# brunothg/sfm-mvs-pipeline

Measured on AMD Instinct MI355X. Metric: descriptor-pairs/s matched, higher is better.
Workload: dtype int8->int32 (exact; f32 in/out); 1 GPU; 50 images x 8192 SIFT-128 f32, unordered all-pairs (1225 pairs); descriptors_per_image=8192, pairs=1225, parallelism=pair-sharded x1

## Files before the change

sfm-mvs-pipeline_amd/csrc/match_device.hpp:

```cpp
#pragma once
#include <hip/hip_runtime.h>
#include <cstdint>
#include <climits>
#include <cstdlib>
#include "match_common.hpp"
#include "sift_fp6.hpp"

namespace sfmx {

typedef int i32x4 __attribute__((ext_vector_type(4)));
typedef int i32x16 __attribute__((ext_vector_type(16)));
typedef unsigned u32x4 __attribute__((ext_vector_type(4)));
typedef int i32x8 __attribute__((ext_vector_type(8)));
typedef float f32x4 __attribute__((ext_vector_type(4)));
typedef float f32x16 __attribute__((ext_vector_type(16)));

#define GLOBAL_AS __attribute__((address_space(1)))
#define LDS_AS __attribute__((address_space(3)))

__device__ __forceinline__ int med3i(int a, int b, int c) { return max(min(a, b), min(max(a, b), c)); }
__device__ __forceinline__ int v_med3(int a, int b, int c) {
    int d;
    asm("v_med3_i32 %0, %1, %2, %3" : "=v"(d) : "v"(a), "v"(b), "v"(c));
    return d;
// ... 154 lines not shown
            }
        }
        if ((s % SPC) == SPC - 1 || s + 1 == nstages) {
            const int cb = (s / SPC) * 256;
#pragma unroll
            for (int qt = 0; qt < QT; ++qt) {
                const int p1 = __shfl_xor(c1[qt], 32), p2 = __shfl_xor(c2[qt], 32);
                const int m1 = max(c1[qt], p1), m2 = max(min(c1[qt], p1), max(c2[qt], p2));
#pragma unroll
                for (int e = 0; e < 2; ++e) {
                    const int key = e == 0 ? m1 : m2;
                    if (key != INT_MIN) {
                        const int t_ = -(key >> 8), j_ = cb + 255 - (key & 255);
                        if (t_ < T2[qt]) {
                            if (t_ < T1[qt]) { T2[qt] = T1[qt]; J2[qt] = J1[qt]; T1[qt] = t_; J1[qt] = j_; }
                            else { T2[qt] = t_; J2[qt] = j_; }
                        }
                    }
                }
                c1[qt] = c2[qt] = INT_MIN;
            }
        }
        asm volatile("s_waitcnt vmcnt(0)" ::: "memory");
        __syncthreads();
    }

#pragma unroll
    for (int qt = 0; qt < QT; ++qt) {
        const int qi = qrow[qt];
        if (h != 0 || qi < 0) continue;
        if constexpr (LISTS) {
            const long long na = norm[L.row0 + qi];
            const unsigned long long k1 = T1[qt] != INT_MAX ? ((unsigned long long)(na + T1[qt]) << 32) | (unsigned)J1[qt] : ~0ull;
            const unsigned long long k2 = T2[qt] != INT_MAX ? ((unsigned long long)(na + T2[qt]) << 32) | (unsigned)J2[qt] : ~0ull;
            *reinterpret_cast<ulonglong2*>(top2 + 2 * (P.dense_base + qslot[qt])) = make_ulonglong2(k1, k2);
            continue;
        }
        const int64_t o = P.dense_base + qi;
        if (nt == 0) { out_idx[o] = -1; out_dist[o] = 0.f; continue; }
        const int64_t na = norm[L.row0 + qi];
        const int64_t s1 = (int64_t)T1[qt] + na, s2 = (int64_t)T2[qt] + na;
        if (nt >= 2 && s2 >= SQRT_SAFE) {
            const int slot = atomicAdd(slow_count, 1);
            slow_list[slot] = make_int2(w.pair, qi);
            out_idx[o] = -2;
            continue;
        }
        const float d1 = sqrt_rn_int(s1);
        out_idx[o] = lowe_select(J1[qt], d1, nt >= 2 ? sqrt_rn_int(s2) : 0.f, nt, ratio);
        out_dist[o] = d1;
    }
}

template <int QT, int WAVES, int MINW, int STAGE, bool MFMA_FIRST, bool GATHER = false, bool LISTS = false, bool VIA = false>
__global__ __launch_bounds__(WAVES * 64, MINW)
void sift_knn2_kernel(const WorkItem* __restrict__ work, const PairDev* __restrict__ pairs,
                      const ImgDev* __restrict__ imgs, const int8_t* __restrict__ desc8,
                      const int32_t* __restrict__ norm, const int32_t* __restrict__ keyc,
                      int32_t* __restrict__ out_idx, float* __restrict__ out_dist,
                      int2* __restrict__ slow_list, int32_t* __restrict__ slow_count, double ratio,
                      const int32_t* __restrict__ qlist = nullptr, const int32_t* __restrict__ qcount = nullptr,
                      const int32_t* __restrict__ work2_n = nullptr, unsigned long long* __restrict__ top2 = nullptr,
                      const int32_t* __restrict__ via = nullptr) {
#define SIFT_KNN2_ITEM(item, nwork)                                                                                    \
    sift_knn2_item<QT, WAVES, MINW, STAGE, MFMA_FIRST, GATHER, LISTS, VIA>(                                            \
        item, nwork, work, pairs, imgs, desc8, norm, keyc, out_idx, out_dist, slow_list, slow_count, ratio, qlist, qcount, \
        top2, via)
    if constexpr (VIA) {
        const int nwork = *work2_n;
        for (int item = blockIdx.x; item < nwork; item += gridDim.x) SIFT_KNN2_ITEM(item, nwork);
    } else if constexpr (GATHER) {
        const int nwork = *work2_n;
        if ((int)blockIdx.x < nwork) SIFT_KNN2_ITEM((int)blockIdx.x, nwork);
    } else {
        SIFT_KNN2_ITEM((int)blockIdx.x, (int)gridDim.x);
    }
#undef SIFT_KNN2_ITEM
}

__device__ __forceinline__ int xcd_ticket(int32_t* ticket, int n) {
    const int x0 = (int)(__builtin_amdgcn_s_getreg(0x1814) & 7);
    for (int k = 0; k < 8; ++k) {
        const int x = (x0 + k) & 7, b0 = (int)((int64_t)n * x / 8), b1 = (int)((int64_t)n * (x + 1) / 8);
        if (b1 <= b0) continue;
        if (__hip_atomic_load(&ticket[x], __ATOMIC_RELAXED, __HIP_MEMORY_SCOPE_AGENT) >= b1 - b0) continue;
        const int t = atomicAdd(&ticket[x], 1);
        if (t < b1 - b0) return b0 + t;
    }
    return -1;
}

template <bool CERT>
__device__ __forceinline__ void screen6_forward(float k1, float k2, int r1, int qi, int nt, int2 q2, int emax2, int amax2,
                                                double ratio, int pair, int64_t dense_base, int32_t* __restrict__ qlist,
                                                int32_t* __restrict__ qcount, int32_t* __restrict__ qmask,
                                                unsigned long long* __restrict__ top2, int32_t* __restrict__ qlist2,
                                                int32_t* __restrict__ qcount2) {
    const int usable = (int)(nt >= 2) & (int)(k2 > fp6::KEY_VALID);
    const int rej = usable & fp6::certainly_rejected(k1, k2, q2.x, q2.y, emax2, amax2, ratio);
    if (rej == 0) {
        const int64_t slot = dense_base + atomicAdd(&qcount[pair], 1);
        qlist[slot] = qi;
        if constexpr (CERT) {
            const int cert = fp6::certified(k1, k2, r1, nt, q2.x, q2.y, emax2, amax2, ratio);
            qmask[slot] = cert ? 1 << r1 : QMASK_FULL_ROUTE;
            if (!cert) qlist2[dense_base + atomicAdd(&qcount2[pair], 1)] = (int32_t)(slot - dense_base);
        } else {
            qmask[slot] = 0xFFFF;
        }
        top2[2 * slot] = ~0ull;
        top2[2 * slot + 1] = ~0ull;
    }
}

template <int STAGE>
struct Screen6Stage {
    static constexpr int WAVES = 4;
    static constexpr int A_BYTES = STAGE * 64, B_BYTES = STAGE * 32;
    static constexpr int GA = A_BYTES / (WAVES * 64 * 16), GB = B_BYTES / (WAVES * 64 * 16), GK = STAGE / 64;
    static constexpr int BUF_BYTES = A_BYTES + B_BYTES + STAGE * 4;
    static_assert(STAGE % 128 == 0 && ROW_ALIGN % STAGE == 0, "whole DMA instructions per wave; stages inside the padded rows");
    __amdgpu_buffer_rsrc_t rows, keys;
    int va, vb, vk;
    int wid;

    __device__ __forceinline__ Screen6Stage(const uint32_t* __restrict__ desc6, const float* __restrict__ keyf, const ImgDev& R) {
        const int tid = threadIdx.x;
        wid = __builtin_amdgcn_readfirstlane(tid >> 6);
        const int ra = tid >> 2, rb = tid >> 1;
        va = ra * fp6::ROW_BYTES + 16 * ((tid & 3) ^ fp6::swz_a(ra));
        vb = rb * fp6::ROW_BYTES + 64 + 16 * ((tid & 1) ^ fp6::swz_b(rb));
        vk = (tid & 63) * 4;
        rows = __builtin_amdgcn_make_buffer_rsrc(const_cast<uint32_t*>(desc6 + R.row0 * fp6::ROW_WORDS), 0,
                                                 R.rows_pad * fp6::ROW_BYTES, 0x00020000);
        keys = __builtin_amdgcn_make_buffer_rsrc(const_cast<float*>(keyf + R.row0), 0, R.rows_pad * 4, 0x00020000);
    }
    __device__ __forceinline__ void issue(char* lds, int s, int buf) const {
        char* base = lds + buf * BUF_BYTES;
        const int row0 = s * STAGE;
#pragma unroll
        for (int i = 0; i < GA; ++i)
            __builtin_amdgcn_raw_ptr_buffer_load_lds(rows, (LDS_AS void*)(base + (i * WAVES + wid) * 1024), 16, va,
                                                     (row0 + i * 64) * fp6::ROW_BYTES, 0, 0);
#pragma unroll
        for (int i = 0; i < GB; ++i)
            __builtin_amdgcn_raw_ptr_buffer_load_lds(rows, (LDS_AS void*)(base + A_BYTES + (i * WAVES + wid) * 1024), 16, vb,
                                                     (row0 + i * 128) * fp6::ROW_BYTES, 0, 0);
        if (wid < GK)
            __builtin_amdgcn_raw_ptr_buffer_load_lds(keys, (LDS_AS void*)(base + A_BYTES + B_BYTES + wid * 256), 4, vk,
                                                     (row0 + wid * 64) * 4, 0, 0);
    }
};

template <int QT, int WAVES, int MINW, int STAGE, bool CERT>
__global__ __launch_bounds__(WAVES * 64, MINW)
void sift_screen6_kernel(const WorkItem* __restrict__ work, const PairDev* __restrict__ pairs,
                         const ImgDev* __restrict__ imgs, const uint32_t* __restrict__ desc6,
                         const float* __restrict__ keyf, const int2* __restrict__ ne,
                         const int32_t* __restrict__ imax,
                         int32_t* __restrict__ qlist, int32_t* __restrict__ qcount, double ratio,
                         int32_t* __restrict__ qmask, unsigned long long* __restrict__ top2,
                         int32_t* __restrict__ qlist2, int32_t* __restrict__ qcount2) {
    static_assert(QT * WAVES * 16 == 512, "work items are 512 queries");
    using Stage = Screen6Stage<STAGE>;
    static_assert(WAVES == Stage::WAVES, "whole DMA instructions per wave");
    constexpr int A_BYTES = Stage::A_BYTES, B_BYTES = Stage::B_BYTES, BUF_BYTES = Stage::BUF_BYTES;
    __shared__ __attribute__((aligned(16))) char lds[2 * BUF_BYTES];

    const int lane = threadIdx.x & 63, g = lane >> 4, l16 = lane & 15;
    const WorkItem w = work[xcd_remap(blockIdx.x, gridDim.x)];
    const PairDev P = pairs[w.pair];
    const ImgDev L = imgs[P.left], R = imgs[P.right];
    const int nq = L.rows, nt = R.rows;
    const Stage stager(desc6, keyf, R);
    const int wid = stager.wid;
    const int qbase = w.q0 + wid * (QT * 16);

    i32x8 bq[QT];
#pragma unroll
    for (int qt = 0; qt < QT; ++qt) {
        const uint32_t* src = desc6 + (L.row0 + qbase + qt * 16 + l16) * fp6::ROW_WORDS;
        const i32x4 lo = *reinterpret_cast<const i32x4*>(src + 4 * g);
        const int2 hi = *reinterpret_cast<const int2*>(src + 16 + 2 * g);
        bq[qt] = i32x8{lo.x, lo.y, lo.z, lo.w, hi.x, hi.y, 0, 0};
    }
    float ch[QT][4];
#pragma unroll
    for (int qt = 0; qt < QT; ++qt)
#pragma unroll
        for (int i = 0; i < 4; ++i) ch[qt][i] = fp6::KEY_INIT;

    const int nstages = (nt + STAGE - 1) / STAGE;
    const char* ra = lds + l16 * 64 + 16 * (g ^ fp6::swz_a(l16));
    const char* rb = lds + A_BYTES + l16 * 32 + 16 * ((g >> 1) ^ fp6::swz_b(l16)) + 8 * (g & 1);
    const char* rk = lds + A_BYTES + B_BYTES + 16 * g;
    static_assert(fp6::swz_a(16) == fp6::swz_a(0) && fp6::swz_b(16) == fp6::swz_b(0), "swizzle period of 16 rows");

    if (nstages > 0) stager.issue(lds, 0, 0);
    asm volatile("s_waitcnt vmcnt(0)" ::: "memory");
    __syncthreads();
    for (int s = 0; s < nstages; ++s) {
        const int buf = s & 1;
        if (s + 1 < nstages) stager.issue(lds, s + 1, buf ^ 1);
        const char *pa = ra + buf * BUF_BYTES, *pb = rb + buf * BUF_BYTES, *pk = rk + buf * BUF_BYTES;
#pragma unroll
        for (int t = 0; t < STAGE / 32; ++t) {
            i32x8 a[2];
            f32x4 cinit[2];
#pragma unroll
            for (int b = 0; b < 2; ++b) {
                const int blk = 2 * t + b;
                const i32x4 lo = *reinterpret_cast<const i32x4*>(pa + blk * 16 * 64);
                const long long hi = *(const volatile LDS_AS long long*)(pb + blk * 16 * 32);
                a[b] = i32x8{lo.x, lo.y, lo.z, lo.w, (int)hi, (int)(hi >> 32), 0, 0};
                cinit[b] = *reinterpret_cast<const f32x4*>(pk + blk * 16 * 4);
            }
#pragma unroll
            for (int qt = 0; qt < QT; ++qt) {
                const f32x4 acc0 = fp6::mfma16<fp6::FMT_E2M3, false>(a[0], bq[qt], cinit[0]);
                const f32x4 acc1 = fp6::mfma16<fp6::FMT_E2M3, false>(a[1], bq[qt], cinit[1]);
#pragma unroll
                for (int i = 0; i < 4; ++i) ch[qt][i] = fmaxf(fmaxf(ch[qt][i], acc0[i]), acc1[i]);
            }
        }
        asm volatile("s_waitcnt vmcnt(0)" ::: "memory");
        __syncthreads();
    }

    const int emax2 = imax[2 * P.right], amax2 = imax[2 * P.right + 1];
    static_assert(QT % 4 == 0, "four tiles per decision pass");
    float kk1[4] = {}, kk2[4] = {};
    int rr1[4] = {};
#pragma unroll
    for (int qt = 0; qt < QT; ++qt) {
        float k1 = fp6::KEY_INIT, k2 = fp6::KEY_INIT;
        int r1 = 4 * g;
#pragma unroll
        for (int i = 0; i < 4; ++i) {
            const float v = ch[qt][i];
            if constexpr (CERT) r1 = v > k1 ? 4 * g + i : r1;
            k2 = fmaxf(k2, fminf(k1, v));
            k1 = fmaxf(k1, v);
        }
#pragma unroll
        for (int o = 16; o <= 32; o <<= 1) {
            const float p1 = __shfl_xor(k1, o), p2 = __shfl_xor(k2, o);
            if constexpr (CERT) {
                const int pr = __shfl_xor(r1, o);
                r1 = p1 > k1 ? pr : r1;
            }
            k2 = fmaxf(fminf(k1, p1), fmaxf(k2, p2));
            k1 = fmaxf(k1, p1);
        }
        kk1[qt & 3] = k1; kk2[qt & 3] = k2; rr1[qt & 3] = r1;
        if ((qt & 3) != 3) continue;
        k1 = kk1[0]; k2 = kk2[0]; r1 = rr1[0];
#pragma unroll
        for (int j = 1; j < 4; ++j) {
            k1 = g == j ? kk1[j] : k1;
            k2 = g == j ? kk2[j] : k2;
            r1 = g == j ? rr1[j] : r1;
        }
        const int qi = qbase + ((qt & ~3) + g) * 16 + l16;
        if (qi >= nq || nt == 0) continue;
        screen6_forward<CERT>(k1, k2, r1, qi, nt, ne[L.row0 + qi], emax2, amax2, ratio, w.pair, P.dense_base, qlist, qcount,
                              qmask, top2, qlist2, qcount2);
    }
}

constexpr int SIFT_RIDE_MAX = 32;

template <int QTMAX>
__global__ __launch_bounds__(256, 4)
void sift_rows_kernel(const PairDev* __restrict__ pairs, const ImgDev* __restrict__ imgs,
                      const int8_t* __restrict__ desc8, const int32_t* __restrict__ norm,
                      const int32_t* __restrict__ qlist, const int32_t* __restrict__ qmask,
                      const int32_t* __restrict__ qcount, const int32_t* __restrict__ qcount2,
                      const int32_t* __restrict__ porder, unsigned long long* __restrict__ top2) {
    constexpr int WIN = 1024;
    constexpr int EPT = WIN / 256;
    constexpr int RIDER = 1 << 30;
    constexpr int TILE = 32 * SIFT_DIM;
    __shared__ __attribute__((aligned(16))) char rows_lds[4][2][TILE];
    __shared__ int nrm_lds[4][2][64];
    __shared__ int pool[WIN];
    __shared__ __attribute__((aligned(16))) int strip[4][32];
    __shared__ int s_cnt[5];
    static_assert(sizeof(rows_lds) + sizeof(nrm_lds) + sizeof(pool) + sizeof(strip) + sizeof(s_cnt) <= 160 * 1024 / 4,
                  "pass-2 LDS must leave four workgroups resident per CU");

    const int tid = threadIdx.x, lane = tid & 63, h = lane >> 5, l32 = lane & 31;
    const int wid = __builtin_amdgcn_readfirstlane(tid >> 6);
    const int item = xcd_remap(blockIdx.x, gridDim.x);
    const int pi = porder[item >> 2], G = item & 3, r = 4 * G + wid;
    const int cnt = qcount[pi];
    if (cnt == 0) return;
    const PairDev P = pairs[pi];
    const ImgDev L = imgs[P.left], R = imgs[P.right];
    const int nt = R.rows;
    if (4 * G >= nt) return;
    const bool live = r < nt;
    const int ntile = R.rows_pad >> 9;
    const int32_t* qls = qlist + P.dense_base;
    const int32_t* qms = qmask + P.dense_base;
    const bool riders = qcount2[pi] <= SIFT_RIDE_MAX;

    const int8_t* rbase = desc8 + (R.row0 + r) * SIFT_DIM;
    const int32_t* nbase = norm + R.row0 + r;
    auto stage = [&](int t, int b) {
        const int8_t* src = rbase + (int64_t)t * (32 * 16 * SIFT_DIM);
#pragma unroll
        for (int u = 0; u < 4; ++u) {
            const int rr = 8 * u + (lane >> 3), c = (lane & 7) ^ ((rr >> 1) & 7);
            __builtin_amdgcn_global_load_lds((const GLOBAL_AS void*)(src + (unsigned)(rr * (16 * SIFT_DIM) + 16 * c)),
                                             (LDS_AS void*)(&rows_lds[wid][b][u * 1024]), 16, 0, 0);
        }
        __builtin_amdgcn_global_load_lds((const GLOBAL_AS void*)(nbase + t * (32 * 16) + 16 * l32),
                                         (LDS_AS void*)(&nrm_lds[wid][b][0]), 4, 0, 0);
    };
    int cur = 0;
    if (live) stage(0, 0);

    for (int e0 = 0; e0 < cnt; e0 += WIN) {
        if (tid < 5) s_cnt[tid] = 0;
        __syncthreads();
        int ent[EPT], at[EPT], li[EPT];
#pragma unroll
        for (int k = 0; k < EPT; ++k) {
            const int e = e0 + k * 256 + tid;
            li[k] = -1;
            ent[k] = at[k] = 0;
            if (e < cnt) {
                const int mk = qms[e];
                if (mk & QMASK_FULL_ROUTE) li[k] = riders ? 4 : -1;
                else if (mk != 0 && ((__ffs(mk) - 1) >> 2) == G) li[k] = (__ffs(mk) - 1) & 3;
                if (li[k] >= 0) {
                    ent[k] = qls[e] | ((e - e0) << 20) | (li[k] == 4 ? RIDER : 0);
                    at[k] = atomicAdd(&s_cnt[li[k]], 1);
                }
            }
        }
        __syncthreads();
        int base[5], n_l[5];
        base[0] = 0;
#pragma unroll
        for (int l = 0; l < 5; ++l) {
            n_l[l] = __builtin_amdgcn_readfirstlane(s_cnt[l]);
            if (l < 4) base[l + 1] = base[l] + n_l[l];
        }
#pragma unroll
        for (int k = 0; k < EPT; ++k)
            if (li[k] >= 0) pool[base[li[k]] + at[k]] = ent[k];
        __syncthreads();
        const int n_own = n_l[wid], b_own = base[wid], n = live ? n_own + n_l[4] : 0;
        for (int g0 = 0; g0 < n; g0 += 32 * QTMAX) {
            const int nqt = min(QTMAX, (n - g0 + 31) >> 5);
            auto entry = [&](int qt) {
                const int qe = g0 + qt * 32 + l32;
                return qe < n ? (qe < n_own ? pool[b_own + qe] : pool[base[4] + qe - n_own]) : -1;
            };
            i32x4 bq[QTMAX][4];
#pragma unroll
            for (int qt = 0; qt < QTMAX; ++qt) {
#pragma unroll
                for (int m = 0; m < 4; ++m) bq[qt][m] = i32x4{0, 0, 0, 0};
                if (qt < nqt) {
                    const int qpk = entry(qt);
                    const int64_t lrow = L.row0 + (qpk < 0 ? 0 : (qpk & 0xFFFFF));
                    const i32x4* src = reinterpret_cast<const i32x4*>(desc8 + lrow * SIFT_DIM);
#pragma unroll
                    for (int m = 0; m < 4; ++m) bq[qt][m] = src[2 * m + h];
                }
            }
            int T1[QTMAX], T2[QTMAX], c1[QTMAX], c2[QTMAX];
            unsigned JJ[QTMAX];
#pragma unroll
            for (int qt = 0; qt < QTMAX; ++qt) {
                T1[qt] = T2[qt] = INT_MAX; JJ[qt] = 0; c1[qt] = c2[qt] = INT_MIN;
            }
            for (int t = 0; t < ntile; ++t) {
// ... 317 lines not shown
```

sfm-mvs-pipeline_amd/csrc/match_diag.hip:

```cpp
#ifdef SFMX_DIAG
#include "match_device.hpp"
#include "diag.hpp"

namespace sfmx {

__global__ void prep_hamming_kernel(const uint8_t* __restrict__ src, int rows, int cols, int rows_pad,
                                    uint8_t* __restrict__ dst) {
    const int64_t i = (int64_t)blockIdx.x * blockDim.x + threadIdx.x;
    const int64_t total = (int64_t)rows_pad * ORB_BYTES;
    if (i >= total) return;
    const int r = (int)(i / ORB_BYTES), c = (int)(i % ORB_BYTES);
    dst[i] = (r < rows && c < cols) ? src[(int64_t)r * cols + c] : 0;
}

template <int QT, int WAVES, int MINW, int STAGE>
__global__ __launch_bounds__(WAVES * 64, MINW)
void sift_screen_kernel(const WorkItem* __restrict__ work, const PairDev* __restrict__ pairs,
                        const ImgDev* __restrict__ imgs, const int8_t* __restrict__ desc8,
                        const int32_t* __restrict__ norm, const int32_t* __restrict__ keyc2,
                        int32_t* __restrict__ out_idx, float* __restrict__ out_dist,
                        int32_t* __restrict__ qlist, int32_t* __restrict__ qcount, double ratio) {
    constexpr int GLDS = STAGE * SIFT_DIM / (WAVES * 64 * 16);
    static_assert(GLDS * WAVES * 64 * 16 == STAGE * SIFT_DIM, "stage must split into whole 16-B pieces");
    constexpr int DESC_BYTES = STAGE * SIFT_DIM;
// ... 872 lines not shown
                    for (int r = 0; r < 4; r += 2) {
                        const float ka = acc[b][r], kb = acc[b][r + 1];
                        c2[qt] = fmaxf(__builtin_amdgcn_fmed3f(c1[qt], ka, kb), c2[qt]);
                        c1[qt] = fmaxf(c1[qt], fmaxf(ka, kb));
                    }
            }
        }
        if ((s % SPC) == SPC - 1 || s + 1 == nstages) {
            const int cb = (s / SPC) * CHUNK;
#pragma unroll
            for (int qt = 0; qt < QT; ++qt) {
                float m1 = c1[qt], m2 = c2[qt];
#pragma unroll
                for (int o = 16; o <= 32; o <<= 1) {
                    const float p1 = __shfl_xor(m1, o), p2 = __shfl_xor(m2, o);
                    m2 = fmaxf(fminf(m1, p1), fmaxf(m2, p2));
                    m1 = fmaxf(m1, p1);
                }
#pragma unroll
                for (int e = 0; e < 2; ++e) {
                    const float v = e == 0 ? m1 : m2;
                    if (v >= KEY_FLOOR) {
                        const float ip = __builtin_floorf(v);
                        const int dot = (int)ip - 767;
                        const int t_ = (256 - dot) >> 1;
                        const int j_ = cb + 16383 - (int)((v - ip) * 16384.0f);
                        if (t_ < T2[qt]) {
                            if (t_ < T1[qt]) { T2[qt] = T1[qt]; J2[qt] = J1[qt]; T1[qt] = t_; J1[qt] = j_; }
                            else { T2[qt] = t_; J2[qt] = j_; }
                        }
                    }
                }
                c1[qt] = c2[qt] = 0.f;
            }
        }
        asm volatile("s_waitcnt vmcnt(0)" ::: "memory");
        __syncthreads();
    }
#pragma unroll
    for (int qt = 0; qt < QT; ++qt) {
        const int qi = qrow[qt];
        if (g != 0 || qi < 0) continue;
        const int64_t o = P.dense_base + qi;
        if (nt == 0) { out_idx[o] = -1; out_dist[o] = 0.f; continue; }
        const float d1 = (float)T1[qt], d2 = (float)T2[qt];
        out_idx[o] = lowe_select(J1[qt], d1, d2, nt, ratio);
        out_dist[o] = d1;
    }
}

template <int QPL>
__global__ __launch_bounds__(256, 2)
void orb_knn2_kernel(const WorkItem* __restrict__ work, const PairDev* __restrict__ pairs,
                     const ImgDev* __restrict__ imgs, const uint8_t* __restrict__ desc8,
                     int32_t* __restrict__ out_idx, float* __restrict__ out_dist, double ratio) {
    constexpr int STAGE = 256;
    constexpr int BUF = STAGE * ORB_BYTES;
    __shared__ __attribute__((aligned(16))) uint8_t lds[2 * BUF];
    const int wid = threadIdx.x >> 6;
    const WorkItem w = work[xcd_remap(blockIdx.x, gridDim.x)];
    const PairDev P = pairs[w.pair];
    const ImgDev L = imgs[P.left], R = imgs[P.right];
    const int nq = L.rows, nt = R.rows;

    u32x4 q[QPL][2];
#pragma unroll
    for (int e = 0; e < QPL; ++e) {
        const int qi = w.q0 + e * 256 + threadIdx.x;
        const u32x4* src = reinterpret_cast<const u32x4*>(desc8 + (L.row0 + qi) * ORB_BYTES);
        q[e][0] = src[0]; q[e][1] = src[1];
    }
    unsigned b1[QPL], b2[QPL];
#pragma unroll
    for (int e = 0; e < QPL; ++e) b1[e] = b2[e] = 0xffffffffu;

    const uint8_t* tbase = desc8 + R.row0 * ORB_BYTES;
    const int nstages = (nt + STAGE - 1) / STAGE;
    auto stage = [&](int s, int buf) {
        uint8_t* base = lds + buf * BUF;
#pragma unroll
        for (int i = 0; i < 2; ++i) {
            const uint8_t* g = tbase + (int64_t)s * BUF + i * 4096 + threadIdx.x * 16;
            __builtin_amdgcn_global_load_lds((const GLOBAL_AS void*)g, (LDS_AS void*)(base + i * 4096 + wid * 1024), 16, 0, 0);
        }
    };
    if (nstages > 0) stage(0, 0);
    asm volatile("s_waitcnt vmcnt(0)" ::: "memory");
    __syncthreads();
    for (int s = 0; s < nstages; ++s) {
        const int buf = s & 1;
        if (s + 1 < nstages) stage(s + 1, buf ^ 1);
        const u32x4* tl = reinterpret_cast<const u32x4*>(lds + buf * BUF);
        const int lim = min(STAGE, nt - s * STAGE);
        const unsigned j0 = (unsigned)(s * STAGE);
        for (int jj = 0; jj < lim; ++jj) {
            const u32x4 t0 = tl[2 * jj], t1 = tl[2 * jj + 1];
#pragma unroll
            for (int e = 0; e < QPL; ++e) {
                unsigned d = __builtin_popcount(q[e][0].x ^ t0.x);
                d += __builtin_popcount(q[e][0].y ^ t0.y);
                d += __builtin_popcount(q[e][0].z ^ t0.z);
                d += __builtin_popcount(q[e][0].w ^ t0.w);
                d += __builtin_popcount(q[e][1].x ^ t1.x);
                d += __builtin_popcount(q[e][1].y ^ t1.y);
                d += __builtin_popcount(q[e][1].z ^ t1.z);
                d += __builtin_popcount(q[e][1].w ^ t1.w);
                const unsigned key = (d << 23) | (j0 + jj);
                b2[e] = med3u(b1[e], b2[e], key);
                b1[e] = min(b1[e], key);
            }
        }
        asm volatile("s_waitcnt vmcnt(0)" ::: "memory");
        __syncthreads();
    }
#pragma unroll
    for (int e = 0; e < QPL; ++e) {
        const int qi = w.q0 + e * 256 + threadIdx.x;
        if (qi >= nq) continue;
        const int64_t o = P.dense_base + qi;
        if (nt == 0) { out_idx[o] = -1; out_dist[o] = 0.f; continue; }
        const float d1 = (float)(b1[e] >> 23), d2 = (float)(b2[e] >> 23);
        out_idx[o] = lowe_select((int)(b1[e] & 0x7fffffu), d1, d2, nt, ratio);
        out_dist[o] = d1;
    }
}

hipError_t launch_prep_hamming(const uint8_t* src, int rows, int cols, int rows_pad, uint8_t* dst, hipStream_t st) {
    const int64_t total = (int64_t)rows_pad * ORB_BYTES;
    if (total == 0) return hipSuccess;
    prep_hamming_kernel<<<(unsigned)((total + 255) / 256), 256, 0, st>>>(src, rows, cols, rows_pad, dst);
    return hipGetLastError();
}
#define RECORD_SCREEN()                                              \
    if (ev_screen) {    \
        const hipError_t e_ = hipEventRecord(ev_screen, st);         \
        if (e_ != hipSuccess) return e_;                             \
    }

hipError_t launch_sift_diag(const MatchRoute& r, const MatchBufs& b, int n_work, int n_pairs, double ratio, hipStream_t st,
                            hipEvent_t ev_screen) {
    if (r.sift_product()) return launch_sift_product(b, n_work, n_pairs, ratio, r.full_row_grid, st, ev_screen);
    if (n_work == 0) return hipSuccess;
    using R = MatchRoute;
    int32_t* qlist2 = reinterpret_cast<int32_t*>(b.slot1);
    int32_t* qcount2 = b.qcount + arena_qcount2(n_pairs);
    if (r.sift_lists) {
        switch (r.pass2) {
        case R::ROWS:
        case R::SUBSET_CERT:
            if (r.screen == R::FP6_32)
                sift_screen6w_kernel<4, 2, 128, true><<<n_work, 256, 0, st>>>(b.work, b.pairs, b.imgs, b.desc6, b.keyf, b.ne, b.imax,
                                                                             b.qlist, b.qcount, ratio, b.qmask, b.top2, qlist2, qcount2);
            else
                sift_screen6_kernel<8, 4, 2, 128, true><<<n_work, 256, 0, st>>>(b.work, b.pairs, b.imgs, b.desc6, b.keyf, b.ne, b.imax,
                                                                               b.qlist, b.qcount, ratio, b.qmask, b.top2, qlist2, qcount2);
            RECORD_SCREEN();
            if (r.pass2 == R::SUBSET_CERT)
                sift_subset_kernel<4, true><<<n_pairs * 16, 256, 0, st>>>(b.pairs, b.imgs, b.desc8, b.norm, b.qlist, b.qmask, b.qcount,
                                                                          b.porder, b.top2, b.slot1, qcount2, SIFT_RIDE_MAX);
            else
                sift_rows_kernel<2><<<n_pairs * 4, 256, 0, st>>>(b.pairs, b.imgs, b.desc8, b.norm, b.qlist, b.qmask, b.qcount, qcount2,
                                                                 b.porder, b.top2);
            return launch_sift_full_rows(b, n_work, n_pairs, ratio, r.full_row_grid, st);
        case R::FULL_ROWS:
            sift_screen6_kernel<8, 4, 2, 128, false><<<n_work, 256, 0, st>>>(b.work, b.pairs, b.imgs, b.desc6, b.keyf, b.ne, b.imax,
                                                                            b.qlist, b.qcount, ratio, b.qmask, b.top2, nullptr, nullptr);
            RECORD_SCREEN();
            compact_work_kernel<7><<<1, 1024, 0, st>>>(b.porder, n_pairs, b.qcount, b.work2, b.work2_n);
            sift_knn2_kernel<1, 4, 2, 128, false, true, true><<<n_work << 2, 256, 0, st>>>(
                b.work2, b.pairs, b.imgs, b.desc8, b.norm, b.keyc, nullptr, nullptr, nullptr, nullptr, ratio, b.qlist, b.qcount,
                b.work2_n, b.top2);
            return hipGetLastError();
        case R::SUBSET:
            sift_screen16_kernel<8, 4, 2, 64, true, false, true><<<n_work, 256, 0, st>>>(
                b.work, b.pairs, b.imgs, b.desc8, b.norm, b.keyc2, b.dense_idx, b.dense_dist, b.qlist, b.qcount, ratio, b.qmask, b.top2);
            RECORD_SCREEN();
            sift_subset_kernel<4, true><<<n_pairs * 16, 256, 0, st>>>(b.pairs, b.imgs, b.desc8, b.norm, b.qlist, b.qmask, b.qcount,
                                                                      b.porder, b.top2, b.slot1);
            return hipGetLastError();
        default: return hipErrorInvalidValue;
        }
    }
    if (r.pass2 == R::SUBSET) {
        static const int slots = resident_slots(sift_screen16_kernel<8, 4, 2, 64, true, true>, 256);
        if (slots > 0 && r.persist)
            sift_screen16_kernel<8, 4, 2, 64, true, true><<<std::min(n_work, slots), 256, 0, st>>>(
                b.work, b.pairs, b.imgs, b.desc8, b.norm, b.keyc2, b.dense_idx, b.dense_dist, b.qlist, b.qcount, ratio, b.qmask,
                b.top2, b.qcount + n_pairs, n_work);
        else
            sift_screen16_kernel<8, 4, 2, 64, true><<<n_work, 256, 0, st>>>(b.work, b.pairs, b.imgs, b.desc8, b.norm, b.keyc2,
                                                                           b.dense_idx, b.dense_dist, b.qlist, b.qcount, ratio,
                                                                           b.qmask, b.top2);
        RECORD_SCREEN();
        sift_subset_kernel<4><<<n_pairs * 16, 256, 0, st>>>(b.pairs, b.imgs, b.desc8, b.norm, b.qlist, b.qmask, b.qcount, b.porder,
                                                            b.top2, b.slot1);
        sift_settle_kernel<<<n_pairs, 256, 0, st>>>(b.pairs, b.imgs, b.qlist, b.qcount, b.top2, b.dense_idx, b.dense_dist,
                                                    b.slow_list, b.slow_count, ratio, b.qmask, b.slot1);
        return hipGetLastError();
    }
    if (r.pass2 == R::GATHER) {
#define SCREEN_ARGS b.work, b.pairs, b.imgs, b.desc8, b.norm, b.keyc2, b.dense_idx, b.dense_dist, b.qlist, b.qcount, ratio
        switch (r.screen) {
        case R::INT8_32: sift_screen_kernel<4, 4, 2, 64><<<n_work, 256, 0, st>>>(SCREEN_ARGS); break;
        case R::INT8_16: sift_screen16_kernel<8, 4, 2, 64><<<n_work, 256, 0, st>>>(SCREEN_ARGS); break;
        case R::INT8_16_S128: sift_screen16_kernel<8, 4, 2, 128><<<n_work, 256, 0, st>>>(SCREEN_ARGS); break;
        case R::INT8_16_W8: sift_screen16_kernel<4, 8, 2, 64><<<n_work, 512, 0, st>>>(SCREEN_ARGS); break;
        default: return hipErrorInvalidValue;
        }
#undef SCREEN_ARGS
        RECORD_SCREEN();
#define PASS2_LAUNCH(ISH, QT, W)                                                                                 \
    static_assert((1 << (ISH)) == (QT) * (W) * 32, "pass-2 item size must equal the queries one block covers");  \
    static_assert((ISH) >= 7 && (ISH) <= 9, "work2 holds n_work << 2 items: items of 128..512 queries");         \
    compact_work_kernel<ISH><<<1, 1024, 0, st>>>(b.porder, n_pairs, b.qcount, b.work2, b.work2_n);               \
    sift_knn2_kernel<QT, W, 2, 128, false, true><<<n_work << (9 - ISH), W * 64, 0, st>>>(                         \
        b.work2, b.pairs, b.imgs, b.desc8, b.norm, b.keyc, b.dense_idx, b.dense_dist, b.slow_list, b.slow_count, ratio, \
        b.qlist, b.qcount, b.work2_n)
        switch (r.p2_qt * r.p2_waves) {
        case 4: PASS2_LAUNCH(7, 1, 4); break;
        case 8:
            if (r.p2_waves == 4) { PASS2_LAUNCH(8, 2, 4); }
            else { PASS2_LAUNCH(8, 4, 2); }
            break;
        case 16: PASS2_LAUNCH(9, 4, 4); break;
        default: return hipErrorInvalidValue;
        }
#undef PASS2_LAUNCH
        return hipGetLastError();
    }
#define SIFT_LAUNCH(QT, W, MINW, ST, MF)                                                                       \
    sift_knn2_kernel<QT, W, MINW, ST, MF><<<n_work, W * 64, 0, st>>>(b.work, b.pairs, b.imgs, b.desc8, b.norm, b.keyc, \
                                                                     b.dense_idx, b.dense_dist, b.slow_list, b.slow_count, ratio)
    switch (r.pass2) {
    case R::SINGLE: SIFT_LAUNCH(4, 4, 2, 128, false); break;
    case R::SINGLE_MINW1: SIFT_LAUNCH(4, 4, 1, 128, false); break;
    case R::SINGLE_R01: SIFT_LAUNCH(2, 8, 1, 64, true); break;
    default: return hipErrorInvalidValue;
    }
#undef SIFT_LAUNCH
    return hipGetLastError();
}

hipError_t launch_two_pass_overlap(bool sift, const MatchBatch* batches, int nb, const MatchBufs& b, int n_pairs, double ratio,
                                   hipStream_t st, hipEvent_t ev_screen, const OverlapStreams& os) {
    hipError_t e;
    const uint8_t* desc4 = reinterpret_cast<const uint8_t*>(b.desc8);
#define OCHK(x) do { if ((e = (x)) != hipSuccess) return e; } while (0)
    OCHK(hipEventRecord(os.start, st));
    OCHK(hipStreamWaitEvent(os.sx, os.start, 0));
    OCHK(hipStreamWaitEvent(os.sp, os.start, 0));
    for (int i = 0; i < nb; ++i) {
        const MatchBatch& B = batches[i];
        hipStream_t s = (i & 1) ? os.sx : st;
        if (B.nw == 0) {}
        else if (sift)
            sift_screen16_kernel<8, 4, 2, 64, true><<<B.nw, 256, 0, s>>>(b.work + B.w0, b.pairs, b.imgs, b.desc8, b.norm, b.keyc2,
                                                                         b.dense_idx, b.dense_dist, b.qlist, b.qcount, ratio,
                                                                         b.qmask, b.top2);
        else
            orb_screen16_kernel<8, 4, 2, 64, true><<<B.nw, 256, 0, s>>>(b.work + B.w0, b.pairs, b.imgs, desc4, b.keyc, b.dense_idx,
                                                                        b.dense_dist, b.qlist, b.qcount, ratio, b.qmask, b.top2);
        OCHK(hipGetLastError());
        OCHK(hipEventRecord(os.screen[i], s));
        OCHK(hipStreamWaitEvent(os.sp, os.screen[i], 0));
        if (sift) {
            sift_subset_kernel<4><<<B.np * 16, 256, 0, os.sp>>>(b.pairs, b.imgs, b.desc8, b.norm, b.qlist, b.qmask, b.qcount,
                                                                b.porder + B.p0, b.top2, b.slot1);
            sift_settle_kernel<<<B.np, 256, 0, os.sp>>>(b.pairs, b.imgs, b.qlist, b.qcount, b.top2, b.dense_idx, b.dense_dist,
                                                        b.slow_list, b.slow_count, ratio, b.qmask, b.slot1, b.porder + B.p0);
        } else {
            OCHK(launch_orb_pass2(b, b.porder + B.p0, B.np, b.porder + B.p0, ratio, os.sp));
        }
        OCHK(hipGetLastError());
    }
    OCHK(hipEventRecord(os.sx_done, os.sx));
    OCHK(hipStreamWaitEvent(st, os.sx_done, 0));
    if (ev_screen) OCHK(hipEventRecord(ev_screen, st));
    OCHK(hipEventRecord(os.sp_done, os.sp));
    OCHK(hipStreamWaitEvent(st, os.sp_done, 0));
#undef OCHK
    return hipSuccess;
}

hipError_t launch_sift_slow(const MatchBufs& b, double ratio, hipStream_t st) {
    sift_slow_kernel<<<256, 256, 0, st>>>(b.slow_list, b.slow_count, b.pairs, b.imgs, b.desc8, b.norm, b.dense_idx, b.dense_dist,
                                          ratio);
    return hipGetLastError();
}

hipError_t launch_orb_diag(const MatchRoute& r, const MatchBufs& b, int n_work, int n_pairs, double ratio, hipStream_t st,
                           hipEvent_t ev_screen) {
    if (r.orb_product()) return launch_orb_product(b, n_work, n_pairs, ratio, st, ev_screen);
    if (n_work == 0) return hipSuccess;
    using R = MatchRoute;
    const uint8_t* desc = reinterpret_cast<const uint8_t*>(b.desc8);
    if (r.orb == R::ORB_VALU) {
        orb_knn2_kernel<2><<<n_work, 256, 0, st>>>(b.work, b.pairs, b.imgs, desc, b.dense_idx, b.dense_dist, ratio);
        return hipGetLastError();
    }
    if (r.orb == R::ORB_SUBSET) {
        static const int slots = resident_slots(orb_screen16_kernel<8, 4, 2, 64, true, true>, 256);
        if (slots > 0 && r.persist)
            orb_screen16_kernel<8, 4, 2, 64, true, true><<<std::min(n_work, slots), 256, 0, st>>>(
                b.work, b.pairs, b.imgs, desc, b.keyc, b.dense_idx, b.dense_dist, b.qlist, b.qcount, ratio, b.qmask, b.top2,
                b.qcount + n_pairs, n_work);
        else
            orb_screen16_kernel<8, 4, 2, 64, true><<<n_work, 256, 0, st>>>(b.work, b.pairs, b.imgs, desc, b.keyc, b.dense_idx,
                                                                          b.dense_dist, b.qlist, b.qcount, ratio, b.qmask, b.top2);
        RECORD_SCREEN();
        return launch_orb_pass2(b, b.porder, n_pairs, nullptr, ratio, st);
    }
#define ORB_PASS2(ISH, QT, W)                                                                                   \
    static_assert((1 << (ISH)) == (QT) * (W) * 16, "pass-2 item size must equal the queries one block covers"); \
    static_assert((ISH) >= 7 && (ISH) <= 9, "work2 holds n_work << 2 items: items of 128..512 queries");       \
    orb_screen16_kernel<8, 4, 2, 64><<<n_work, 256, 0, st>>>(b.work, b.pairs, b.imgs, desc, b.keyc, b.dense_idx, b.dense_dist, \
                                                              b.qlist, b.qcount, ratio);                        \
    RECORD_SCREEN();                                                                                            \
    compact_work_kernel<ISH><<<1, 1024, 0, st>>>(b.porder, n_pairs, b.qcount, b.work2, b.work2_n);              \
// ... 27 lines not shown
```

sfm-mvs-pipeline_amd/csrc/match_kernels.hip:

```cpp
#include "match_device.hpp"

namespace sfmx {

struct Fp6Rows {
    uint32_t* desc6;
    float* keyf;
    int2* ne;
};
__device__ __forceinline__ int2 prep_l2_row(const float* __restrict__ src, int r, int rows, int cols,
                                            int8_t* __restrict__ dst, int32_t* __restrict__ norm,
                                            int32_t* __restrict__ keyc, int32_t* __restrict__ keyc2,
                                            int32_t* __restrict__ nonintegral, const Fp6Rows* f6 = nullptr);
constexpr int PREP_ROWS = 64;
static_assert(ROW_ALIGN % PREP_ROWS == 0 && PREP_ROWS % 8 == 0, "whole 8-row steps, no partial workgroup");
__global__ void prep_l2_batch_kernel(const PrepImg* __restrict__ tab, int8_t* __restrict__ desc8,
                                     int32_t* __restrict__ norm, int32_t* __restrict__ keyc,
                                     int32_t* __restrict__ keyc2, int32_t* __restrict__ flags, Fp6Rows f6,
                                     int32_t* __restrict__ imax) {
    const PrepImg t = tab[blockIdx.y];
    const Fp6Rows f6i{f6.desc6 + t.row0 * fp6::ROW_WORDS, f6.keyf + t.row0, f6.ne + t.row0};
    int emax = 0, amax = 0;
    for (int r = blockIdx.x * PREP_ROWS + (threadIdx.x >> 5); r < min((int)(blockIdx.x + 1) * PREP_ROWS, t.rows_pad);
         r += blockDim.x >> 5) {
        const int2 em = prep_l2_row(t.src, r, t.rows, t.cols, desc8 + t.row0 * SIFT_DIM, norm + t.row0, keyc + t.row0,
// ... 494 lines not shown
        for (int i = tid; i < words; i += 1024) acc += __popc(bits[i] & ~bits[words + i]);
    }
#pragma unroll
    for (int o = 32; o > 0; o >>= 1) { acc += __shfl_xor(acc, o); bad += __shfl_xor(bad, o); }
    if (lane == 0) { sh[wid] = acc; sh[16 + wid] = bad; }
    __syncthreads();
    if (tid == 0) {
        int run = 0, b = 0;
        for (int i = 0; i < 16; ++i) { run += sh[i]; b += sh[16 + i]; }
        if (b) atomicAdd(unsettled, b);
        if (n_slow) atomicAdd(slow_count, n_slow);
        counts[R.pair] = run;
        keep[R.pair] = run < min_count ? 0 : 1;
    }
}

__global__ __launch_bounds__(1024)
void assemble_lists_kernel(const PairRec* __restrict__ recs, const int32_t* __restrict__ qlist,
                           const int32_t* __restrict__ qcount, const unsigned long long* __restrict__ top2,
                           const int32_t* __restrict__ out_idx, const float* __restrict__ out_dist, int distinct,
                           const int64_t* __restrict__ counts, const int64_t* __restrict__ offsets,
                           DMatchDev* __restrict__ out) {
    extern __shared__ __attribute__((aligned(16))) unsigned bits[];
    __shared__ int sh[32];
    const int tid = threadIdx.x, lane = tid & 63, wid = tid >> 6;
    const PairRec R = recs[blockIdx.x];
    const int words = (R.nt + 31) >> 5;
    if (!R.lists) {
        const int32_t* ix = out_idx + R.dense_base;
        if (distinct) dense_dup_bits(bits, ix, R.nq, words);
        dense_write(bits, sh, ix, out_dist + R.dense_base, R.nq, words, distinct, offsets[R.pair], out);
        return;
    }
    const int cnt = qcount[R.pair];
    if (cnt == 0 || counts[R.pair] == 0) return;
    const int W = (R.nq + 31) >> 5;
    unsigned* bm = bits;
    unsigned* pre = bits + W;
    unsigned* seen = bits + 2 * W;
    for (int i = tid; i < W; i += 1024) bm[i] = 0;
    if (distinct)
        for (int i = tid; i < 2 * words; i += 1024) seen[i] = 0;
    __syncthreads();
    const int32_t* qls = qlist + R.dense_base;
    const int2* res = reinterpret_cast<const int2*>(top2 + 2 * R.dense_base);
    if (distinct) {
        for (int e = tid; e < cnt; e += 1024) {
            const int j = res[2 * e].x;
            if (j >= 0) mark_seen(seen, words, j);
        }
        __syncthreads();
    }
    for (int e = tid; e < cnt; e += 1024) {
        const int j = res[2 * e].x;
        if (j >= 0 && !(distinct && ((seen[words + (j >> 5)] >> (j & 31)) & 1u))) {
            const int qi = qls[e];
            atomicOr(&bm[qi >> 5], 1u << (qi & 31));
        }
    }
    __syncthreads();
    {
        const int per = (W + 1023) / 1024, w0 = min(tid * per, W), w1 = min(w0 + per, W);
        int mine = 0;
        for (int w = w0; w < w1; ++w) mine += __popc(bm[w]);
        int incl = mine;
        for (int o = 1; o < 64; o <<= 1) {
            const int v = __shfl_up(incl, o);
            if (lane >= o) incl += v;
        }
        if (lane == 63) sh[wid] = incl;
        __syncthreads();
        int at = incl - mine;
        for (int i = 0; i < wid; ++i) at += sh[i];
        for (int w = w0; w < w1; ++w) { pre[w] = at; at += __popc(bm[w]); }
    }
    __syncthreads();
    DMatchDev* o = out + offsets[R.pair];
    for (int e = tid; e < cnt; e += 1024) {
        const int2 r = res[2 * e];
        if (r.x >= 0 && !(distinct && ((seen[words + (r.x >> 5)] >> (r.x & 31)) & 1u))) {
            const int qi = qls[e];
            const unsigned below = bm[qi >> 5] & ((1u << (qi & 31)) - 1u);
            o[pre[qi >> 5] + __popc(below)] = DMatchDev{qi, r.x, 0, __int_as_float(r.y)};
        }
    }
}

__global__ __launch_bounds__(1024)
void scan_offsets_kernel(const int64_t* __restrict__ counts, int n, int64_t* __restrict__ offsets) {
    __shared__ long long sh[1024];
    long long run = 0;
    for (int c0 = 0; c0 < n; c0 += 1024) {
        const int i = c0 + threadIdx.x;
        const long long v = i < n ? counts[i] : 0;
        sh[threadIdx.x] = v;
        __syncthreads();
        for (int o = 1; o < 1024; o <<= 1) {
            const long long y = threadIdx.x >= o ? sh[threadIdx.x - o] : 0;
            __syncthreads();
            sh[threadIdx.x] += y;
            __syncthreads();
        }
        if (i < n) offsets[i] = run + sh[threadIdx.x] - v;
        run += sh[1023];
        __syncthreads();
    }
    if (threadIdx.x == 0) offsets[n] = run;
}

__global__ void selftest_sqrt_kernel(int64_t n, uint32_t* __restrict__ out) {
    const int64_t i = (int64_t)blockIdx.x * blockDim.x + threadIdx.x;
    if (i < n) out[i] = __float_as_uint(sqrt_rn_int(i));
}

hipError_t launch_selftest_sqrt(int64_t n, uint32_t* out, hipStream_t st) {
    if (n <= 0) return hipSuccess;
    selftest_sqrt_kernel<<<(unsigned)((n + 255) / 256), 256, 0, st>>>(n, out);
    return hipGetLastError();
}
hipError_t launch_prep_f32(const float* src, int rows, int cols, int rows_pad, float* dst, hipStream_t st) {
    const int64_t total = (int64_t)rows_pad * SIFT_DIM;
    if (total == 0) return hipSuccess;
    prep_f32_kernel<<<(unsigned)((total + 255) / 256), 256, 0, st>>>(src, rows, cols, rows_pad, dst);
    return hipGetLastError();
}

hipError_t launch_prep_hamming_fp4(const uint8_t* src, int rows, int cols, int rows_pad, uint8_t* dst, int32_t* keyc,
                                   hipStream_t st) {
    if (rows_pad == 0) return hipSuccess;
    prep_hamming_fp4_kernel<<<(rows_pad + 7) / 8, 256, 0, st>>>(src, rows, cols, rows_pad,
                                                               reinterpret_cast<uint32_t*>(dst), keyc);
    return hipGetLastError();
}

constexpr int SIFT_ROWS_QT = 2;
constexpr int SIFT_FULL_ROW_SLOTS = 1024;

hipError_t launch_sift_full_rows(const MatchBufs& b, int n_work, int n_pairs, double ratio, int full_row_grid, hipStream_t st) {
    const int32_t* qlist2 = reinterpret_cast<const int32_t*>(b.slot1);
    const int32_t* qcount2 = b.qcount + arena_qcount2(n_pairs);
    compact_work_kernel<7><<<1, 1024, 0, st>>>(b.porder, n_pairs, qcount2, b.work2, b.work2_n, SIFT_RIDE_MAX);
    static const int slots = resident_slots(sift_knn2_kernel<1, 4, 2, 128, false, true, true, true>, 256);
    const int grid = std::min(n_work << 2, full_row_grid > 0 ? full_row_grid : 2 * (slots > 0 ? slots : SIFT_FULL_ROW_SLOTS));
    sift_knn2_kernel<1, 4, 2, 128, false, true, true, true><<<grid, 256, 0, st>>>(
        b.work2, b.pairs, b.imgs, b.desc8, b.norm, b.keyc, nullptr, nullptr, nullptr, nullptr, ratio, b.qlist, qcount2,
        b.work2_n, b.top2, qlist2);
    return hipGetLastError();
}
hipError_t launch_sift_product(const MatchBufs& b, int n_work, int n_pairs, double ratio, int full_row_grid, hipStream_t st,
                               hipEvent_t ev_screen) {
    if (n_work == 0) return hipSuccess;
    int32_t* qlist2 = reinterpret_cast<int32_t*>(b.slot1);
    int32_t* qcount2 = b.qcount + arena_qcount2(n_pairs);
    sift_screen6_kernel<8, 4, 2, 128, true><<<n_work, 256, 0, st>>>(b.work, b.pairs, b.imgs, b.desc6, b.keyf, b.ne, b.imax,
                                                                   b.qlist, b.qcount, ratio, b.qmask, b.top2, qlist2, qcount2);
    if (ev_screen) {
        const hipError_t e = hipEventRecord(ev_screen, st);
        if (e != hipSuccess) return e;
    }
    sift_rows_kernel<SIFT_ROWS_QT><<<n_pairs * 4, 256, 0, st>>>(b.pairs, b.imgs, b.desc8, b.norm, b.qlist, b.qmask, b.qcount,
                                                                 qcount2, b.porder, b.top2);
    return launch_sift_full_rows(b, n_work, n_pairs, ratio, full_row_grid, st);
}
hipError_t launch_orb_pass2(const MatchBufs& b, const int32_t* porder, int np, const int32_t* settle_order, double ratio,
                            hipStream_t st) {
    const uint8_t* desc4 = reinterpret_cast<const uint8_t*>(b.desc8);
    orb_subset_kernel<4, 2><<<np * 16, 256, 0, st>>>(b.pairs, b.imgs, desc4, b.qlist, b.qmask, b.qcount, porder, b.top2);
    orb_settle_kernel<<<np, 256, 0, st>>>(b.pairs, b.imgs, b.qlist, b.qcount, b.top2, b.dense_idx, b.dense_dist, ratio,
                                          settle_order);
    return hipGetLastError();
}
hipError_t launch_orb_product(const MatchBufs& b, int n_work, int n_pairs, double ratio, hipStream_t st, hipEvent_t ev_screen) {
    if (n_work == 0) return hipSuccess;
    const uint8_t* desc4 = reinterpret_cast<const uint8_t*>(b.desc8);
    orb_screen16_kernel<8, 4, 2, 64, true><<<n_work, 256, 0, st>>>(b.work, b.pairs, b.imgs, desc4, b.keyc, b.dense_idx,
                                                                  b.dense_dist, b.qlist, b.qcount, ratio, b.qmask, b.top2);
    if (ev_screen) {
        const hipError_t e = hipEventRecord(ev_screen, st);
        if (e != hipSuccess) return e;
    }
    return launch_orb_pass2(b, b.porder, n_pairs, nullptr, ratio, st);
}
hipError_t launch_sift_f32(const MatchBufs& b, int n_work32, double ratio, hipStream_t st) {
    if (n_work32 == 0) return hipSuccess;
    sift_f32_kernel<<<n_work32, 512, 0, st>>>(b.work32, nullptr, b.pairs, b.imgs, b.f32, b.dense_idx, b.dense_dist, ratio);
    return hipGetLastError();
}
hipError_t launch_assemble(const MatchBufs& b, int n_pairs, int distinct, int min_count, int max_nt, hipStream_t st) {
    if (n_pairs == 0) {
        (void)hipMemsetAsync(b.offsets, 0, sizeof(int64_t), st);
        return hipGetLastError();
    }
    const size_t shmem = distinct ? (size_t)2 * ((max_nt + 31) / 32) * 4 : 0;
    if (shmem > 150 * 1024) return hipErrorInvalidValue;
    assemble_kernel<0><<<n_pairs, 1024, shmem, st>>>(b.pairs, b.imgs, b.dense_idx, b.dense_dist, distinct, min_count, b.counts,
                                                     b.keep, nullptr, nullptr, b.unsettled);
    scan_offsets_kernel<<<1, 1024, 0, st>>>(b.counts, n_pairs, b.offsets);
    assemble_kernel<1><<<n_pairs, 1024, shmem, st>>>(b.pairs, b.imgs, b.dense_idx, b.dense_dist, distinct, min_count, b.counts,
                                                     b.keep, b.offsets, b.out, b.unsettled);
    return hipGetLastError();
}
hipError_t launch_finish_lists(const MatchBufs& b, int n_pairs, double ratio, int distinct, int min_count, int max_nq,
                               int max_nt, hipStream_t st, hipEvent_t ev_main) {
    hipError_t e;
    if (n_pairs == 0) {
        (void)hipMemsetAsync(b.offsets, 0, sizeof(int64_t), st);
        if ((e = hipGetLastError()) != hipSuccess) return e;
        return ev_main ? hipEventRecord(ev_main, st) : hipSuccess;
    }
    const size_t dup = distinct ? (size_t)2 * ((max_nt + 31) / 32) * 4 : 0;
    const size_t shmem = (size_t)2 * ((max_nq + 31) / 32) * 4 + dup;
    if (shmem > 150 * 1024) return hipErrorInvalidValue;
    sift_finish_kernel<<<n_pairs, 1024, dup, st>>>(b.recs, b.qlist, b.qmask, b.qcount, b.top2, b.slot1, b.slow_list,
                                                   b.slow_count, b.desc8, b.norm, b.dense_idx, ratio, distinct, min_count,
                                                   b.counts, b.keep, b.unsettled);
    if ((e = hipGetLastError()) != hipSuccess) return e;
    if (ev_main && (e = hipEventRecord(ev_main, st)) != hipSuccess) return e;
    scan_offsets_kernel<<<1, 1024, 0, st>>>(b.counts, n_pairs, b.offsets);
    assemble_lists_kernel<<<n_pairs, 1024, shmem, st>>>(b.recs, b.qlist, b.qcount, b.top2, b.dense_idx, b.dense_dist, distinct,
                                                        b.counts, b.offsets, b.out);
    return hipGetLastError();
}

}
```

Baseline: 18960 billion descriptor-pairs/s.

## Software-pipeline LDS reads in screen6 kernel with pinned register double-sets

```diff
diff --git a/sfm-mvs-pipeline_amd/csrc/match_device.hpp b/sfm-mvs-pipeline_amd/csrc/match_device.hpp
--- a/sfm-mvs-pipeline_amd/csrc/match_device.hpp
+++ b/sfm-mvs-pipeline_amd/csrc/match_device.hpp
@@ -330,6 +330,55 @@
     }
 };
 
+typedef int i32x2 __attribute__((ext_vector_type(2)));
+#define SCREEN6_REGS_0(C) C "{v[120:123]}"(lo0), C "{v[124:125]}"(hi0), C "{v[132:135]}"(k0), C "{v[126:129]}"(lo1), C "{v[130:131]}"(hi1), C "{v[136:139]}"(k1)
+#define SCREEN6_REGS_1(C) C "{v[140:143]}"(lo0), C "{v[144:145]}"(hi0), C "{v[152:155]}"(k0), C "{v[146:149]}"(lo1), C "{v[150:151]}"(hi1), C "{v[156:159]}"(k1)
+template <int SET, int T>
+__device__ __forceinline__ void screen6_request(i32x4& lo0, i32x2& hi0, f32x4& k0, i32x4& lo1, i32x2& hi1, f32x4& k1,
+                                                unsigned pa, unsigned pb, unsigned pk) {
+#define SCREEN6_REQUEST(REGS)                                                                                           \
+    asm volatile("ds_read_b128 %0, %6 offset:%9\n\t"                                                                    \
+                 "ds_read_b64 %1, %7 offset:%10\n\t"                                                                    \
+                 "ds_read_b128 %2, %8 offset:%11\n\t"                                                                   \
+                 "ds_read_b128 %3, %6 offset:%12\n\t"                                                                   \
+                 "ds_read_b64 %4, %7 offset:%13\n\t"                                                                    \
+                 "ds_read_b128 %5, %8 offset:%14"                                                                        \
+                 : REGS("=")                                                                                            \
+                 : "v"(pa), "v"(pb), "v"(pk), "n"(2 * T * 1024), "n"(2 * T * 512), "n"(2 * T * 64),                      \
+                   "n"((2 * T + 1) * 1024), "n"((2 * T + 1) * 512), "n"((2 * T + 1) * 64)                                \
+                 : "memory")
+    if constexpr (SET == 0) SCREEN6_REQUEST(SCREEN6_REGS_0);
+    else SCREEN6_REQUEST(SCREEN6_REGS_1);
+#undef SCREEN6_REQUEST
+}
+template <int SET, int N>
+__device__ __forceinline__ void screen6_arrived(i32x4& lo0, i32x2& hi0, f32x4& k0, i32x4& lo1, i32x2& hi1, f32x4& k1) {
+    if constexpr (SET == 0) asm volatile("s_waitcnt lgkmcnt(%6)" : SCREEN6_REGS_0("+") : "n"(N));
+    else asm volatile("s_waitcnt lgkmcnt(%6)" : SCREEN6_REGS_1("+") : "n"(N));
+}
+template <int QT>
+__device__ __forceinline__ void screen6_mul(const i32x8 (&bq)[QT], float (&ch)[QT][4], i32x4 lo0, i32x2 hi0, f32x4 k0,
+                                            i32x4 lo1, i32x2 hi1, f32x4 k1) {
+    __builtin_amdgcn_sched_barrier(0);
+    const i32x8 a0 = i32x8{lo0.x, lo0.y, lo0.z, lo0.w, hi0.x, hi0.y, 0, 0};
+    const i32x8 a1 = i32x8{lo1.x, lo1.y, lo1.z, lo1.w, hi1.x, hi1.y, 0, 0};
+#pragma unroll
+    for (int qt = 0; qt < QT; ++qt) {
+        const f32x4 acc0 = fp6::mfma16<fp6::FMT_E2M3, false>(a0, bq[qt], k0);
+        const f32x4 acc1 = fp6::mfma16<fp6::FMT_E2M3, false>(a1, bq[qt], k1);
+#pragma unroll
+        for (int i = 0; i < 4; ++i) ch[qt][i] = fmaxf(fmaxf(ch[qt][i], acc0[i]), acc1[i]);
+    }
+    __builtin_amdgcn_sched_group_barrier(0x8, 2, 0);
+#pragma unroll
+    for (int qt = 1; qt < QT; ++qt) {
+        __builtin_amdgcn_sched_group_barrier(0x8, 2, 0);
+        __builtin_amdgcn_sched_group_barrier(0x2, 4, 0);
+    }
+    __builtin_amdgcn_sched_group_barrier(0x2, 4, 0);
+    __builtin_amdgcn_sched_barrier(0);
+}
+
 template <int QT, int WAVES, int MINW, int STAGE, bool CERT>
 __global__ __launch_bounds__(WAVES * 64, MINW)
 void sift_screen6_kernel(const WorkItem* __restrict__ work, const PairDev* __restrict__ pairs,
@@ -369,41 +418,46 @@
         for (int i = 0; i < 4; ++i) ch[qt][i] = fp6::KEY_INIT;
 
     const int nstages = (nt + STAGE - 1) / STAGE;
-    const char* ra = lds + l16 * 64 + 16 * (g ^ fp6::swz_a(l16));
-    const char* rb = lds + A_BYTES + l16 * 32 + 16 * ((g >> 1) ^ fp6::swz_b(l16)) + 8 * (g & 1);
-    const char* rk = lds + A_BYTES + B_BYTES + 16 * g;
+    const unsigned lds0 = (unsigned)(size_t)(LDS_AS const void*)lds;
+    const unsigned ra = lds0 + l16 * 64 + 16 * (g ^ fp6::swz_a(l16));
+    const unsigned rb = lds0 + A_BYTES + l16 * 32 + 16 * ((g >> 1) ^ fp6::swz_b(l16)) + 8 * (g & 1);
+    const unsigned rk = lds0 + A_BYTES + B_BYTES + 16 * g;
     static_assert(fp6::swz_a(16) == fp6::swz_a(0) && fp6::swz_b(16) == fp6::swz_b(0), "swizzle period of 16 rows");
+    static_assert(STAGE == 128, "the row loop is written out for four 32-row blocks per stage");
+
+#define SCREEN6_SET0 lo00, hi00, k00, lo01, hi01, k01
+#define SCREEN6_SET1 lo10, hi10, k10, lo11, hi11, k11
 
     if (nstages > 0) stager.issue(lds, 0, 0);
     asm volatile("s_waitcnt vmcnt(0)" ::: "memory");
     __syncthreads();
+    i32x4 lo00, lo01, lo10, lo11;
+    i32x2 hi00, hi01, hi10, hi11;
+    f32x4 k00, k01, k10, k11;
+    unsigned pa = ra, pb = rb, pk = rk;
+    screen6_request<0, 0>(SCREEN6_SET0, pa, pb, pk);
     for (int s = 0; s < nstages; ++s) {
-        const int buf = s & 1;
-        if (s + 1 < nstages) stager.issue(lds, s + 1, buf ^ 1);
-        const char *pa = ra + buf * BUF_BYTES, *pb = rb + buf * BUF_BYTES, *pk = rk + buf * BUF_BYTES;
-#pragma unroll
-        for (int t = 0; t < STAGE / 32; ++t) {
-            i32x8 a[2];
-            f32x4 cinit[2];
-#pragma unroll
-            for (int b = 0; b < 2; ++b) {
-                const int blk = 2 * t + b;
-                const i32x4 lo = *reinterpret_cast<const i32x4*>(pa + blk * 16 * 64);
-                const long long hi = *(const volatile LDS_AS long long*)(pb + blk * 16 * 32);
-                a[b] = i32x8{lo.x, lo.y, lo.z, lo.w, (int)hi, (int)(hi >> 32), 0, 0};
-                cinit[b] = *reinterpret_cast<const f32x4*>(pk + blk * 16 * 4);
-            }
-#pragma unroll
-            for (int qt = 0; qt < QT; ++qt) {
-                const f32x4 acc0 = fp6::mfma16<fp6::FMT_E2M3, false>(a[0], bq[qt], cinit[0]);
-                const f32x4 acc1 = fp6::mfma16<fp6::FMT_E2M3, false>(a[1], bq[qt], cinit[1]);
-#pragma unroll
-                for (int i = 0; i < 4; ++i) ch[qt][i] = fmaxf(fmaxf(ch[qt][i], acc0[i]), acc1[i]);
-            }
-        }
+        if (s + 1 < nstages) stager.issue(lds, s + 1, (s + 1) & 1);
+        screen6_request<1, 1>(SCREEN6_SET1, pa, pb, pk);
+        screen6_arrived<0, 6>(SCREEN6_SET0);
+        screen6_mul<QT>(bq, ch, SCREEN6_SET0);
+        screen6_request<0, 2>(SCREEN6_SET0, pa, pb, pk);
+        screen6_arrived<1, 6>(SCREEN6_SET1);
+        screen6_mul<QT>(bq, ch, SCREEN6_SET1);
+        screen6_request<1, 3>(SCREEN6_SET1, pa, pb, pk);
+        screen6_arrived<0, 6>(SCREEN6_SET0);
+        screen6_mul<QT>(bq, ch, SCREEN6_SET0);
+        screen6_arrived<1, 0>(SCREEN6_SET1);
         asm volatile("s_waitcnt vmcnt(0)" ::: "memory");
         __syncthreads();
-    }
+        const int nb = s & 1 ? -BUF_BYTES : BUF_BYTES;
+        pa += nb; pb += nb; pk += nb;
+        screen6_request<0, 0>(SCREEN6_SET0, pa, pb, pk);
+        screen6_mul<QT>(bq, ch, SCREEN6_SET1);
+    }
+    screen6_arrived<0, 0>(SCREEN6_SET0);
+#undef SCREEN6_SET0
+#undef SCREEN6_SET1
 
     const int emax2 = imax[2 * P.right], amax2 = imax[2 * P.right + 1];
     static_assert(QT % 4 == 0, "four tiles per decision pass");
diff --git a/sfm-mvs-pipeline_amd/csrc/match_diag.hip b/sfm-mvs-pipeline_amd/csrc/match_diag.hip
--- a/sfm-mvs-pipeline_amd/csrc/match_diag.hip
+++ b/sfm-mvs-pipeline_amd/csrc/match_diag.hip
@@ -1048,7 +1048,7 @@
                 sift_screen6w_kernel<4, 2, 128, true><<<n_work, 256, 0, st>>>(b.work, b.pairs, b.imgs, b.desc6, b.keyf, b.ne, b.imax,
                                                                              b.qlist, b.qcount, ratio, b.qmask, b.top2, qlist2, qcount2);
             else
-                sift_screen6_kernel<8, 4, 2, 128, true><<<n_work, 256, 0, st>>>(b.work, b.pairs, b.imgs, b.desc6, b.keyf, b.ne, b.imax,
+                sift_screen6_kernel<8, 4, 3, 128, true><<<n_work, 256, 0, st>>>(b.work, b.pairs, b.imgs, b.desc6, b.keyf, b.ne, b.imax,
                                                                                b.qlist, b.qcount, ratio, b.qmask, b.top2, qlist2, qcount2);
             RECORD_SCREEN();
             if (r.pass2 == R::SUBSET_CERT)
@@ -1059,7 +1059,7 @@
                                                                  b.porder, b.top2);
             return launch_sift_full_rows(b, n_work, n_pairs, ratio, r.full_row_grid, st);
         case R::FULL_ROWS:
-            sift_screen6_kernel<8, 4, 2, 128, false><<<n_work, 256, 0, st>>>(b.work, b.pairs, b.imgs, b.desc6, b.keyf, b.ne, b.imax,
+            sift_screen6_kernel<8, 4, 3, 128, false><<<n_work, 256, 0, st>>>(b.work, b.pairs, b.imgs, b.desc6, b.keyf, b.ne, b.imax,
                                                                             b.qlist, b.qcount, ratio, b.qmask, b.top2, nullptr, nullptr);
             RECORD_SCREEN();
             compact_work_kernel<7><<<1, 1024, 0, st>>>(b.porder, n_pairs, b.qcount, b.work2, b.work2_n);
diff --git a/sfm-mvs-pipeline_amd/csrc/match_kernels.hip b/sfm-mvs-pipeline_amd/csrc/match_kernels.hip
--- a/sfm-mvs-pipeline_amd/csrc/match_kernels.hip
+++ b/sfm-mvs-pipeline_amd/csrc/match_kernels.hip
@@ -670,7 +670,7 @@
     if (n_work == 0) return hipSuccess;
     int32_t* qlist2 = reinterpret_cast<int32_t*>(b.slot1);
     int32_t* qcount2 = b.qcount + arena_qcount2(n_pairs);
-    sift_screen6_kernel<8, 4, 2, 128, true><<<n_work, 256, 0, st>>>(b.work, b.pairs, b.imgs, b.desc6, b.keyf, b.ne, b.imax,
+    sift_screen6_kernel<8, 4, 3, 128, true><<<n_work, 256, 0, st>>>(b.work, b.pairs, b.imgs, b.desc6, b.keyf, b.ne, b.imax,
                                                                    b.qlist, b.qcount, ratio, b.qmask, b.top2, qlist2, qcount2);
     if (ev_screen) {
         const hipError_t e = hipEventRecord(ev_screen, st);
```

Measured after the change: 19260 billion descriptor-pairs/s (median of 6 runs). 1.6% higher.
